# sara-nl/2D-VQ-AE-2

Hardware: AMD Instinct MI355X
Metric: patches/sec (VQAE.forward: encoder -> VQ -> decoder) (higher is better)
Workload: dtype f32; 1 GPU; BASELINE configs[1] (cfg B): batch 256/GPU of 256x256x3 fp32 -> 32x32 codes, K=256, D=128, full forward; global_batch=256, parallelism=patch-sharded x1

## Files before the change

2d-vq-ae-2_amd/csrc/handle.hip:

```cpp
#include "kernels.h"

#include <algorithm>
#include <cmath>
#include <cstdlib>
#include <map>
#include <mutex>
#include <set>
#include <string>
#include <unordered_map>
#include <utility>
#include <vector>

namespace vqae {
char* last_error_buf() {
    static thread_local char buf[512] = {0};
    return buf;
}

ProfState& prof_state() {
    static ProfState p;
    return p;
}

int set_max_dynamic_lds(const void* kernel, int bytes) {
// ... 100 lines not shown
    std::vector<void*> owned;
    float* buf[4] = {nullptr, nullptr, nullptr, nullptr};
    size_t buf_floats = 0;
    void* vq_ws = nullptr;
    size_t vq_ws_bytes = 0;
    float* loss_scratch = nullptr;
    int device = 0;
    bool has_encoder = false, has_decoder = false;
    bool fuse_trunk = true;
    bool t1_ready = false;
    bool up_conv_first = true;
    bool fuse_down = true;
    bool fuse_down16 = true;
    bool fuse_up16 = true;
    bool fuse_up_tail = true;
    bool use_wino = true;
    bool w43_split = true;
    void* idx_scratch = nullptr;
    size_t idx_scratch_bytes = 0;
    float* se_ws = nullptr;
    size_t se_ws_bytes = 0;
    size_t se_gate_off = 0;
};

namespace {

using TensorMap = std::unordered_map<std::string, const vqae_tensor*>;

int find(const TensorMap& tm, const std::string& name, int64_t numel, const float** out) {
    auto it = tm.find(name);
// ... 73 lines not shown
    const int dt = h->cfg.compute_dtype;
    const bool f32 = dt == VQAE_DT_F32, same = mode == MODE_SAME && cout == cin;
    int rc;
#define S_(field, nm) if ((rc = scalar(tm, pre + "." nm, &b->field))) return rc;
    S_(b1a, "bias1a") S_(b1b, "bias1b") S_(b2a, "bias2a") S_(b2b, "bias2b") S_(b3a, "bias3a") S_(b3b, "bias3b")
    S_(b4, "bias4") S_(scale, "scale")
    const bool wino = same && h->use_wino && vqae::wino_trunk_channels(cin, dt);
    const bool wino43 = wino && f32 && vqae::wino43_enabled() && vqae::wino43_channels(cin);
    const bool split = wino43 && h->w43_split && vqae::wino43_split_supported(cin);
    const bool tail = wino || (same && vqae::conv_trunk_tail_channels(cin));
    const bool trunk16 = same && !f32 && vqae::trunk16_channels(cin);
    const bool same8 = same && !f32 && vqae::same8_16_channels(cin);
    const bool down = mode == MODE_DOWN && cout == 2 * cin && h->fuse_down && vqae::down_block_channels(cin);
    const bool down16 = mode == MODE_DOWN && cout == 2 * cin && !f32 && h->fuse_down16 && vqae::down16_channels(cin);
    const bool up16 = mode == MODE_UP && cin == 2 * cout && !f32 && h->fuse_up16 && vqae::up16_channels(cin);

    const int k2 = mode == MODE_SAME ? 3 : (mode == MODE_DOWN ? 2 : 1);
    const float* p;
    if ((rc = find(tm, pre + ".branch_conv1.weight", (int64_t)b->br * cin, &p))) return rc;
    if ((rc = upload_packed(h, p, b->br, cin, 1, &b->w1))) return rc;
    if ((rc = find(tm, pre + ".branch_conv2.weight", (int64_t)b->br * b->br * k2 * k2, &p))) return rc;
    if ((rc = upload_packed(h, p, b->br, b->br, k2, &b->w2))) return rc;
    if (wino && (rc = upload_wino(h, p, cin, &b->wU))) return rc;
    if (wino43 && (rc = upload_wino43(h, p, cin, false, (void**)&b->wU43))) return rc;
    if (split && (rc = upload_wino43(h, p, cin, true, &b->wU43s))) return rc;
    if ((rc = find(tm, pre + ".branch_conv3.weight", (int64_t)cout * b->br, &p))) return rc;
    if ((rc = upload_packed(h, p, cout, b->br, 1, &b->w3))) return rc;
    if (mode != MODE_SAME) {
        S_(b1c, "bias1c") S_(b1d, "bias1d")
        const int ks = mode == MODE_DOWN ? 2 : 1;
// ... 15 lines not shown
    };
    auto pack_t16 = [&](const float* src, int taps, void** dst) {
        if (int r = dev_alloc(h, vqae::trunk16_weight_bytes(cin, taps), dst)) return r;
        return vqae::pack16_weight(src, cin, taps * cin, dt, *dst, nullptr);
    };
    auto pack_r16 = [&](const float* src, int rows, int K, void** dst) {
        if (int r = dev_alloc(h, vqae::down16_weight_bytes(rows, K), dst)) return r;
        return vqae::pack16_weight(src, rows, K, dt, *dst, nullptr);
    };
    if (tail && ((rc = frag_tail(b->w1, &b->w1f)) || (rc = frag_tail(b->w3, &b->w3f)))) return rc;
    if (split && ((rc = split3(b->w1, &b->w1s)) || (rc = split3(b->w3, &b->w3s)))) return rc;
    if (trunk16 && ((rc = pack_t16(b->w1, 1, &b->w1h)) || (rc = pack_t16(b->w2, 9, &b->w2h)) || (rc = pack_t16(b->w3, 1, &b->w3h)))) return rc;
    if (same8 && ((rc = pack_r16(b->w2, 8, 72, &b->w2h)) || (rc = pack_r16(b->w3, 8, 8, &b->w3h)))) return rc;
    if (down && ((rc = frag_rect(b->w1, cin, &b->w1f)) || (rc = frag_rect(b->w2, 4 * cout, &b->w2f)) ||
                 (rc = frag_rect(b->w3, cout, &b->w3f)) || (rc = frag_rect(b->wskip, 4 * cin, &b->wskf)))) return rc;
    if (down16 && ((rc = pack_r16(b->w1, cout, cin, &b->w1h)) || (rc = pack_r16(b->w2, cout, 4 * cout, &b->w2h)) ||
                   (rc = pack_r16(b->w3, cout, cout, &b->w3h)) || (rc = pack_r16(b->wskip, cout, 4 * cin, &b->wskh)))) return rc;
    if (up16 && ((rc = pack_t16(b->w1, 1, &b->w1h)) || (rc = pack_r16(b->w2, cin, cin, &b->w2h)) ||
                 (rc = pack_r16(b->w3, cout, cin, &b->w3h)) || (rc = pack_r16(b->wskip, cout, cin, &b->wskh)))) return rc;
    VQAE_HIP_CHECK(hipDeviceSynchronize());
    return VQAE_OK;
}

int bn_fold(const TensorMap& tm, const std::string& pre, int c, float eps, std::vector<float>* g, std::vector<float>* shift) {
    const float *gamma, *beta, *mean, *var;
    int rc;
    if ((rc = find(tm, pre + ".weight", c, &gamma)) || (rc = find(tm, pre + ".bias", c, &beta)) ||
        (rc = find(tm, pre + ".running_mean", c, &mean)) || (rc = find(tm, pre + ".running_var", c, &var))) return rc;
    g->resize(c); shift->resize(c);
    for (int i = 0; i < c; ++i) {
// ... 252 lines not shown
        out = R;
        break;
    case R_DOWN_FUSED:
        if ((rc = vqae::down_block(X, b.w1f, b.w2f, b.w3f, b.wskf, B, H, W, b.cin, b, dt, R, st))) return rc;
        out = R;
        break;
    case R_DOWN:
        if ((rc = conv(ConvCall(h, B, H, W, b.cin, b.cout, 2, 2, 0, VQAE_PAD_NONE).pre(VQAE_PRE_BIAS, b.b1c, 0.f).bias(b.b1d), X, b.wskip, nullptr, R, st))) return rc;
        if ((rc = run_conv1(h, b, B, H, W, X, P, st))) return rc;
        if ((rc = conv(ConvCall(h, B, H, W, b.br, b.br, 2, 2, 0, VQAE_PAD_NONE).act(b.b3a, b.b3b), P, b.w2, nullptr, Q, st))) return rc;
        if ((rc = conv(ConvCall(h, B, H / 2, W / 2, b.br, b.cout, 1, 1, 0, VQAE_PAD_NONE).scale_bias(b.scale, b.b4), Q, b.w3, R, R, st))) return rc;
        out = R;
        break;
    case R_UP_CONV_FIRST_TAIL:
    case R_UP_CONV_FIRST: {
        const ConvCall sk = ConvCall(h, B, H, W, b.cin, b.cout, 1, 1, 0, VQAE_PAD_NONE).pre(VQAE_PRE_BIAS, b.b1c, 0.f).bias(b.b1d);
        const ConvCall c2(h, B, H, W, b.br, b.br, 1, 1, 0, VQAE_PAD_NONE);
        if ((rc = conv(sk, X, b.wskip, nullptr, Q, st))) return rc;
        if (r == R_UP_CONV_FIRST_TAIL) {
            if ((rc = run_conv1(h, b, B, H, W, X, P, st))) return rc;
            if ((rc = conv(c2, P, b.w2, nullptr, R, st))) return rc;
            if ((rc = vqae::up_tail(R, Q, b.w3, B, H, W, b.br, b.cout, b.b3a, b.b3b, b.scale, b.b4, X, st))) return rc;
            break;
        }
        if ((rc = vqae_bicubic_up2_f32(Q, B, H, W, b.cout, 0.f, R, st))) return rc;
        if ((rc = run_conv1(h, b, B, H, W, X, P, st))) return rc;
        if ((rc = conv(c2, P, b.w2, nullptr, Q, st))) return rc;
        if ((rc = vqae_bicubic_up2_f32(Q, B, H, W, b.br, 0.f, P, st))) return rc;
        if ((rc = conv(ConvCall(h, B, 2 * H, 2 * W, b.br, b.cout, 1, 1, 0, VQAE_PAD_NONE).pre(VQAE_PRE_BIAS_ELU_BIAS, b.b3a, b.b3b).scale_bias(b.scale, b.b4),
                       P, b.w3, R, R, st))) return rc;
        out = R;
        break;
    }
    case R_UP16:
        if ((rc = vqae::trunk16_head(X, b.w1h, b.b1a, b.b1b, b.b2a, b.b2b, Q, (int64_t)B * H * W, b.cin, dt, true, st))) return rc;
        if ((rc = vqae::up16_block(X, Q, b.w2h, b.w3h, b.wskh, B, H, W, b.cin, b, dt, R, st))) return rc;
        out = R;
        break;
    default:
        if ((rc = vqae_bicubic_up2_f32(X, B, H, W, b.cin, b.b1c, P, st))) return rc;
        if ((rc = conv(ConvCall(h, B, 2 * H, 2 * W, b.cin, b.cout, 1, 1, 0, VQAE_PAD_NONE).bias(b.b1d), P, b.wskip, nullptr, R, st))) return rc;
        if ((rc = run_conv1(h, b, B, H, W, X, Q, st))) return rc;
        if ((rc = vqae_bicubic_up2_f32(Q, B, H, W, b.br, 0.f, P, st))) return rc;
        if ((rc = conv(ConvCall(h, B, 2 * H, 2 * W, b.br, b.br, 1, 1, 0, VQAE_PAD_NONE).act(b.b3a, b.b3b), P, b.w2, nullptr, Q, st))) return rc;
        if ((rc = conv(ConvCall(h, B, 2 * H, 2 * W, b.br, b.cout, 1, 1, 0, VQAE_PAD_NONE).scale_bias(b.scale, b.b4), Q, b.w3, R, R, st))) return rc;
        out = R;
// ... 159 lines not shown
        VQAE_REQUIRE(cfg->compute_dtype == VQAE_DT_F32, VQAE_ERR_UNSUPPORTED, "MBConv blocks run in fp32 only");
        VQAE_REQUIRE(cfg->expand_ratio >= 1 && cfg->se_divisor >= 1 && cfg->bn_eps > 0.f, VQAE_ERR_INVALID,
                     "MBConv: expand_ratio %d, se_divisor %d, bn_eps %g", cfg->expand_ratio, cfg->se_divisor, (double)cfg->bn_eps);
    }
    TensorMap tm;
    for (int i = 0; i < n_tensors; ++i) tm[tensors[i].name] = &tensors[i];

    vqae_handle* h = new vqae_handle();
    h->cfg = *cfg;
    if (hipGetDevice(&h->device) != hipSuccess) { delete h; return vqae::fail(VQAE_ERR_HIP, "hipGetDevice failed"); }
    h->fuse_trunk = vqae::env_int("VQAE_NO_TRUNK_FUSION", 0) == 0;
    h->up_conv_first = vqae::env_int("VQAE_NO_UP_REORDER", 0) == 0;
    h->use_wino = vqae::env_int("VQAE_NO_WINOGRAD", 0) == 0;
    h->w43_split = vqae::env_int("VQAE_W43_SPLIT", 1) != 0;
    h->fuse_up_tail = vqae::env_int("VQAE_NO_UP_TAIL_FUSION", 0) == 0;
    h->fuse_down = vqae::env_int("VQAE_NO_DOWN_FUSION", 0) == 0;
    h->fuse_down16 = vqae::env_int("VQAE_NO_DOWN16", 0) == 0;
    h->fuse_up16 = vqae::env_int("VQAE_NO_UP16", 0) == 0;
    h->fuse_stem16 = vqae::env_int("VQAE_NO_STEM16", 0) == 0;
    h->fuse_vq = vqae::env_int("VQAE_NO_VQ_FUSION", 0) == 0;
    h->C = cfg->stem << cfg->n_down;
    h->D = cfg->projection_dim > 0 ? cfg->projection_dim : h->C;
    h->K = cfg->num_embeddings;
    int rc = VQAE_OK;
    const float* p;
    auto bail = [&](int code) { vqae_destroy(h); return code; };

    const bool has_enc = tm.count("encoder.in_stem.weight") > 0;
    const bool has_dec = tm.count("decoder.out_stem.weight") > 0;
    if (!has_enc && !has_dec) return bail(vqae::fail(VQAE_ERR_NOT_FOUND, "neither encoder.* nor decoder.* tensors given"));
// ... 317 lines not shown
```

2d-vq-ae-2_amd/csrc/kernels.h:

```cpp
#pragma once
#include "common.h"

namespace vqae {

struct FixupScalars {
    float b1a, b1b, b2a, b2b, b3a, b3b, b4, scale, b1c, b1d;
};
static_assert(sizeof(FixupScalars) == 10 * sizeof(float), "FixupScalars is read as float[8] / float[10]");

struct NextConv1 {
    const void* w1 = nullptr;
    const void* w1s = nullptr;
    float b1a = 0.f, b1b = 0.f, b2a = 0.f, b2b = 0.f;
    void* t1_next = nullptr;
};

bool conv_trunk_tail_channels(int c);
int conv_tail_kslice(int dtype, int cin);
int conv_trunk_tail(const vqae_conv_args* a, const float* t1, const float* w2, const float* w3, float t_scale, float t_b4,
                    float* xio, const NextConv1& next, hipStream_t stream);

bool wino_trunk_channels(int c, int dtype);
bool wino_trunk_supported(int c, int h, int w, int dtype);
size_t wino_weight_floats(int c);
// ... 50 lines not shown

bool up16_channels(int c);
bool up16_supported(int c, int h, int w, int dtype);
int up16_block(const float* x, const float* t1, const void* w2h, const void* w3h, const void* wskh, int B, int H, int W, int c,
               const FixupScalars& s, int dtype, float* y, hipStream_t stream);

bool stem16_channels(int c0);
bool stem16_supported(int c0, int h, int w, int dtype);
size_t stem16_weight_bytes(int cin);
int stem16_pack_weight(const float* w_dev, int n_out, int cin, int dtype, void* out_dev, hipStream_t stream);
int istem16(const void* x, int x_kind, const float* mean255, const float* inv_std255, const void* wf, const float* bias, int B,
            int H, int W, int c0, float* y, int dtype, hipStream_t stream);
int ostem16(const float* x, const void* wf, const float* bias, int B, int H, int W, int c, float* y, int y_nchw, int dtype,
            hipStream_t stream);

bool up_tail_supported(int cb, int co);
int up_tail(const float* q, const float* s, const float* w3_packed, int B, int H, int W, int cb, int co, float b3a, float b3b,
            float scale, float b4, float* y, hipStream_t stream);
bool conv_small_k_supported(const vqae_conv_args* a);
int conv_small_k(const vqae_conv_args* a, const float* x, const float* w, const float* bias_vec, const float* residual,
                 float* y, hipStream_t stream);
int conv3x3_direct(const void* x, int x_kind, const float* mean255, const float* inv_std255, const float* w,
                   const float* bias, int B, int H, int W, int cin, int cout, float* y, int y_nchw, int dt,
                   hipStream_t stream);

int unstitch_tiles(const void* grid, int grid_dtype, const int32_t* rc, int n_tiles, int th, int tw, void* tiles,
                   int idx_dtype, int gh, int gw, hipStream_t stream);
int pixels_u8(const float* x, int layout, int B, int H, int W, const int32_t* rc, const float* mean255, const float* std255,
              uint8_t* out, int canvas_h, int canvas_w, hipStream_t stream);
int pixels_u8_level_check(const char* who, int H, int W, int level, bool canvas, int canvas_h, int canvas_w);
int pixels_u8_level(const float* x, int layout, int B, int H, int W, int level, const int32_t* rc, const float* mean255,
                    const float* std255, uint8_t* out, int canvas_h, int canvas_w, hipStream_t stream);

// ... 22 lines not shown
```

2d-vq-ae-2_amd/csrc/misc_kernels.hip:

```cpp
#include "kernels.h"
#include "mfma.h"

namespace {


template <int CIN, int COUT>
__global__ __launch_bounds__(256)
void conv3x3_direct_kernel(const void* __restrict__ xin, int x_kind, Norm3 nrm, const float* __restrict__ w,
                           const float* __restrict__ bias, int B, int H, int W, float* __restrict__ y, int y_nchw,
                           int dt) {
    __shared__ float ws[9 * CIN * COUT + COUT];
    for (int i = threadIdx.x; i < 9 * CIN * COUT; i += 256) {
        const int co = i % COUT, ci = (i / COUT) % CIN, tap = i / (COUT * CIN);
        ws[i] = vqae::round_dt(w[((int64_t)co * CIN + ci) * 9 + tap], dt);
    }
    for (int i = threadIdx.x; i < COUT; i += 256) ws[9 * CIN * COUT + i] = vqae::round_dt(bias[i], dt);
    __syncthreads();

    const int64_t npix = (int64_t)B * H * W;
    const int64_t pix = (int64_t)blockIdx.x * 256 + threadIdx.x;
    if (pix >= npix) return;
    const int hw = H * W;
    const int b = (int)(pix / hw), rem = (int)(pix - (int64_t)b * hw);
    const int oy = rem / W, ox = rem - oy * W;
// ... 109 lines not shown
            if (oy < 0 || oy >= OH) continue;
            const float* wy = a == 0 ? w25 : w75;
#pragma unroll
            for (int c = 0; c < 2; ++c) {
                const int ox = 2 * bj + 1 + c;
                if (ox < 0 || ox >= OW) continue;
                const float4* in = c == 0 ? ho : he;
                float4 out;
                out.x = in[0].x * wy[0]; out.y = in[0].y * wy[0]; out.z = in[0].z * wy[0]; out.w = in[0].w * wy[0];
#pragma unroll
                for (int r = 1; r < 4; ++r) {
                    out.x = out.x + in[r].x * wy[r]; out.y = out.y + in[r].y * wy[r];
                    out.z = out.z + in[r].z * wy[r]; out.w = out.w + in[r].w * wy[r];
                }
                y[(((int64_t)b * OH + oy) * OW + ox) * C4 + c4] = out;
            }
        }
    }
}

template <int CB, int CO>
__global__ __launch_bounds__(256)
void up_tail_kernel(const float4* __restrict__ q, const float4* __restrict__ sk, const float* __restrict__ w3, int B, int H,
                    int W, int tiles_x, int tiles_y, float b3a, float b3b, float scale, float b4, float* __restrict__ y) {
    constexpr int LB = CB + 4, LS = CO + 4, GB = CB / 4, GS = CO / 4, NG = GB + GS;
    constexpr int NTL = (CO + 15) / 16;
    static_assert(CB % 16 == 0 && CO % 4 == 0, "conv3 runs on 16x16x4 MFMA tiles");
    const float w75[4] = {-0.03515625f, 0.26171875f, 0.87890625f, -0.10546875f};
    const float w25[4] = {-0.10546875f, 0.87890625f, 0.26171875f, -0.03515625f};
    __shared__ __attribute__((aligned(16))) float Tb[128 * LB];
    __shared__ __attribute__((aligned(16))) float Ts[128 * LS];
    const int tid = threadIdx.x;
    float4 w3r[NTL][CB / 16];
#pragma unroll
    for (int nt = 0; nt < NTL; ++nt)
#pragma unroll
        for (int s_ = 0; s_ < CB / 16; ++s_) {
            const int co = 16 * nt + (tid & 15);
            w3r[nt][s_] = co < CO ? *reinterpret_cast<const float4*>(w3 + co * CB + 16 * s_ + 4 * ((tid & 63) >> 4)) : make_float4(0.f, 0.f, 0.f, 0.f);
        }
    const int OW = 2 * W, OH = 2 * H;
    const int n_tiles = B * tiles_x * tiles_y;
    for (int tile = blockIdx.x; tile < n_tiles; tile += gridDim.x) {
        const int txi = tile % tiles_x;
        const int tyi = (tile / tiles_x) % tiles_y;
        const int64_t b = tile / (tiles_x * tiles_y);
        const int bi0 = 2 * tyi - 1, bj0 = 16 * txi - 1;
        __syncthreads();
        for (int it = tid; it < 32 * NG; it += 256) {
            const int g = it % NG, blk = it / NG;
            const int bi = bi0 + (blk >> 4), bj = bj0 + (blk & 15);
            const bool branch = g < GB;
            const float4* src = branch ? q : sk;
            const int C4 = branch ? GB : GS, gg = branch ? g : g - GB;
            int xs[4], ys[4];
#pragma unroll
            for (int j = 0; j < 4; ++j) {
                int v = bj - 1 + j; xs[j] = v < 0 ? 0 : (v > W - 1 ? W - 1 : v);
                int u = bi - 1 + j; ys[j] = u < 0 ? 0 : (u > H - 1 ? H - 1 : u);
            }
            float4 ho[4], he[4];
#pragma unroll
            for (int r = 0; r < 4; ++r) {
                const float4* row = src + ((b * H + ys[r]) * W) * C4 + gg;
                float4 v[4];
#pragma unroll
                for (int j = 0; j < 4; ++j) v[j] = row[(int64_t)xs[j] * C4];
                ho[r].x = v[0].x * w25[0]; ho[r].y = v[0].y * w25[0]; ho[r].z = v[0].z * w25[0]; ho[r].w = v[0].w * w25[0];
                he[r].x = v[0].x * w75[0]; he[r].y = v[0].y * w75[0]; he[r].z = v[0].z * w75[0]; he[r].w = v[0].w * w75[0];
#pragma unroll
                for (int j = 1; j < 4; ++j) {
                    ho[r].x = __builtin_fmaf(v[j].x, w25[j], ho[r].x); ho[r].y = __builtin_fmaf(v[j].y, w25[j], ho[r].y);
                    ho[r].z = __builtin_fmaf(v[j].z, w25[j], ho[r].z); ho[r].w = __builtin_fmaf(v[j].w, w25[j], ho[r].w);
                    he[r].x = __builtin_fmaf(v[j].x, w75[j], he[r].x); he[r].y = __builtin_fmaf(v[j].y, w75[j], he[r].y);
                    he[r].z = __builtin_fmaf(v[j].z, w75[j], he[r].z); he[r].w = __builtin_fmaf(v[j].w, w75[j], he[r].w);
                }
            }
#pragma unroll
            for (int a = 0; a < 2; ++a) {
                const float* wy = a == 0 ? w25 : w75;
#pragma unroll
                for (int c = 0; c < 2; ++c) {
                    const float4* in = c == 0 ? ho : he;
                    float4 o;
                    o.x = in[0].x * wy[0]; o.y = in[0].y * wy[0]; o.z = in[0].z * wy[0]; o.w = in[0].w * wy[0];
#pragma unroll
                    for (int r = 1; r < 4; ++r) {
                        o.x = __builtin_fmaf(in[r].x, wy[r], o.x); o.y = __builtin_fmaf(in[r].y, wy[r], o.y);
                        o.z = __builtin_fmaf(in[r].z, wy[r], o.z); o.w = __builtin_fmaf(in[r].w, wy[r], o.w);
                    }
                    const int px = (2 * (blk >> 4) + a) * 32 + 2 * (blk & 15) + c;
                    if (branch) {
                        o.x = vqae::elu_act(o.x + b3a) + b3b; o.y = vqae::elu_act(o.y + b3a) + b3b;
                        o.z = vqae::elu_act(o.z + b3a) + b3b; o.w = vqae::elu_act(o.w + b3a) + b3b;
                        *reinterpret_cast<float4*>(Tb + px * LB + 4 * gg) = o;
                    } else {
                        *reinterpret_cast<float4*>(Ts + px * LS + 4 * gg) = o;
                    }
                }
            }
        }
        __syncthreads();
        {
            const int lane = tid & 63, wv = tid >> 6;
            const int li = lane & 15, q = lane >> 4;
#pragma unroll
            for (int gg = 0; gg < 2; ++gg) {
                const int px = 32 * wv + 16 * gg + li;
                const int oy = 2 * bi0 + 1 + (px >> 5), ox = 2 * bj0 + 1 + (px & 31);
                float4 tb[CB / 16];
#pragma unroll
                for (int s_ = 0; s_ < CB / 16; ++s_) tb[s_] = *reinterpret_cast<const float4*>(Tb + px * LB + 16 * s_ + 4 * q);
#pragma unroll
                for (int nt = 0; nt < NTL; ++nt) {
                    typedef float f32x4_t __attribute__((ext_vector_type(4)));
                    f32x4_t acc = {0.f, 0.f, 0.f, 0.f};
#pragma unroll
                    for (int s_ = 0; s_ < CB / 16; ++s_) {
                        const float4 wv4 = w3r[nt][s_];
                        acc = __builtin_amdgcn_mfma_f32_16x16x4f32(wv4.x, tb[s_].x, acc, 0, 0, 0);
                        acc = __builtin_amdgcn_mfma_f32_16x16x4f32(wv4.y, tb[s_].y, acc, 0, 0, 0);
                        acc = __builtin_amdgcn_mfma_f32_16x16x4f32(wv4.z, tb[s_].z, acc, 0, 0, 0);
                        acc = __builtin_amdgcn_mfma_f32_16x16x4f32(wv4.w, tb[s_].w, acc, 0, 0, 0);
                    }
                    if (oy >= 0 && oy < OH && ox >= 0 && ox < OW && 16 * nt + 4 * q < CO) {
                        const float4 sp = *reinterpret_cast<const float4*>(Ts + px * LS + 16 * nt + 4 * q);
                        float o[4];
                        const float sv[4] = {sp.x, sp.y, sp.z, sp.w};
#pragma unroll
                        for (int e = 0; e < 4; ++e) {
                            float tv = acc[e] * scale;
                            tv = tv + b4;
                            o[e] = tv + sv[e];
                        }
                        *reinterpret_cast<float4*>(y + ((b * OH + oy) * OW + ox) * CO + 16 * nt + 4 * q) = make_float4(o[0], o[1], o[2], o[3]);
                    }
                }
            }
        }
    }
}

__global__ __launch_bounds__(256)
void transpose_kernel(const float* __restrict__ in, int R, int S, float* __restrict__ out) {
    __shared__ float tile[32][33];
    const int64_t base = (int64_t)blockIdx.z * R * S;
    const int s0 = blockIdx.x * 32, r0 = blockIdx.y * 32;
    const int tx = threadIdx.x & 31, ty = threadIdx.x >> 5;
#pragma unroll
    for (int j = 0; j < 32; j += 8) {
        const int r = r0 + ty + j, s = s0 + tx;
        if (r < R && s < S) tile[ty + j][tx] = in[base + (int64_t)r * S + s];
// ... 187 lines not shown
        out[0] += r.x; out[1] += r.y; out[2] += r.z; out[3] += r.w;
    }
    if (p.has_act == VQAE_ACT_SILU) {
#pragma unroll
        for (int e = 0; e < 4; ++e) out[e] = out[e] / (1.0f + expf(-out[e]));
    } else if (p.has_act) {
#pragma unroll
        for (int e = 0; e < 4; ++e) out[e] = vqae::elu_act(out[e] + p.act_a) + p.act_b;
    }
    *reinterpret_cast<float4*>(p.y + o) = make_float4(out[0], out[1], out[2], out[3]);
}

}

namespace vqae {
bool up_tail_supported(int cb, int co) { return (cb == 64 && co == 32) || (cb == 32 && co == 16) || (cb == 16 && co == 8); }

int up_tail(const float* q, const float* s, const float* w3_packed, int B, int H, int W, int cb, int co, float b3a, float b3b,
            float scale, float b4, float* y, hipStream_t stream) {
    VQAE_REQUIRE(q && s && w3_packed && y, VQAE_ERR_INVALID, "up_tail: null pointer");
    VQAE_REQUIRE(up_tail_supported(cb, co), VQAE_ERR_UNSUPPORTED, "up_tail: channels %d -> %d", cb, co);
    if ((int64_t)B * H * W == 0) return VQAE_OK;
    const int tiles_x = (int)ceil_div(W + 1, 16), tiles_y = (int)ceil_div(H + 1, 2);
    const int64_t n_tiles = (int64_t)B * tiles_x * tiles_y;
    VQAE_REQUIRE(n_tiles < (1ll << 31), VQAE_ERR_UNSUPPORTED, "up_tail: too many tiles");
    const unsigned grid = (unsigned)std::min<int64_t>(n_tiles, 256 * 40);
    if (cb == 64) up_tail_kernel<64, 32><<<grid, 256, 0, stream>>>((const float4*)q, (const float4*)s, w3_packed, B, H, W, tiles_x, tiles_y, b3a, b3b, scale, b4, y);
    else if (cb == 32) up_tail_kernel<32, 16><<<grid, 256, 0, stream>>>((const float4*)q, (const float4*)s, w3_packed, B, H, W, tiles_x, tiles_y, b3a, b3b, scale, b4, y);
    else up_tail_kernel<16, 8><<<grid, 256, 0, stream>>>((const float4*)q, (const float4*)s, w3_packed, B, H, W, tiles_x, tiles_y, b3a, b3b, scale, b4, y);
    VQAE_LAUNCH_CHECK();
    return VQAE_OK;
}

bool conv_small_k_supported(const vqae_conv_args* a) {
    return a->cin == 8 && a->pad == 0 && a->ksize == a->stride && (a->ksize == 1 || a->ksize == 2) && a->cout % 4 == 0 &&
           a->cout <= 64 && a->pre_mode <= VQAE_PRE_BIAS_ELU_BIAS && a->in_h % a->ksize == 0 && a->in_w % a->ksize == 0;
}

int conv_small_k(const vqae_conv_args* a, const float* x, const float* w, const float* bias_vec, const float* residual,
                 float* y, hipStream_t stream) {
    SmallK p;
    p.x = x; p.w = w; p.bias_vec = bias_vec; p.residual = residual; p.y = y;
    p.H = a->in_h; p.W = a->in_w; p.Ho = a->in_h / a->ksize; p.Wo = a->in_w / a->ksize; p.cout = a->cout;
    p.M = (int64_t)a->batch * p.Ho * p.Wo;
    p.pre_mode = a->pre_mode; p.has_scale = a->has_scale; p.has_bias_s = a->has_bias_s; p.has_act = a->has_act; p.dt = a->dtype;
    p.pre_a = a->pre_a; p.pre_b = a->pre_b; p.scale = a->scale; p.bias_s = a->bias_s; p.act_a = a->act_a; p.act_b = a->act_b;
    const int64_t threads = p.M * (a->cout / 4);
    if (threads == 0) return VQAE_OK;
// ... 137 lines not shown
```

Measured before the change: 4513 patches/s.

## Fuse up-block head convs into one MFMA kernel and retile up_tail

Adds an up_head kernel that computes the skip 1x1 conv, branch conv1 and conv2 for the up block in one pass. The conv1 output stays in LDS, which removes the intermediate global round-trips and the separate launches. The up_tail kernel moves to a new file and is rewritten to tile by output pixels (8x16), loading an input window into LDS before the bicubic interpolation instead of re-reading neighbours per block. The non-tail path also reorders its buffers so the bicubic upsampling runs on the fused outputs. In exchange it adds more register-heavy kernels and more buffer aliasing, which could go wrong.

```diff
diff --git a/2d-vq-ae-2_amd/csrc/handle.hip b/2d-vq-ae-2_amd/csrc/handle.hip
--- a/2d-vq-ae-2_amd/csrc/handle.hip
+++ b/2d-vq-ae-2_amd/csrc/handle.hip
@@ -138,6 +138,7 @@
     bool fuse_down16 = true;
     bool fuse_up16 = true;
     bool fuse_up_tail = true;
+    bool fuse_up_head = true;
     bool use_wino = true;
     bool w43_split = true;
     void* idx_scratch = nullptr;
@@ -241,6 +242,7 @@
     const bool down = mode == MODE_DOWN && cout == 2 * cin && h->fuse_down && vqae::down_block_channels(cin);
     const bool down16 = mode == MODE_DOWN && cout == 2 * cin && !f32 && h->fuse_down16 && vqae::down16_channels(cin);
     const bool up16 = mode == MODE_UP && cin == 2 * cout && !f32 && h->fuse_up16 && vqae::up16_channels(cin);
+    const bool up_head = mode == MODE_UP && cin == 2 * cout && b->br == cin && f32 && h->up_conv_first && h->fuse_up_head && vqae::up_head_channels(cin);
 
     const int k2 = mode == MODE_SAME ? 3 : (mode == MODE_DOWN ? 2 : 1);
     const float* p;
@@ -286,6 +288,8 @@
     if (same8 && ((rc = pack_r16(b->w2, 8, 72, &b->w2h)) || (rc = pack_r16(b->w3, 8, 8, &b->w3h)))) return rc;
     if (down && ((rc = frag_rect(b->w1, cin, &b->w1f)) || (rc = frag_rect(b->w2, 4 * cout, &b->w2f)) ||
                  (rc = frag_rect(b->w3, cout, &b->w3f)) || (rc = frag_rect(b->wskip, 4 * cin, &b->wskf)))) return rc;
+    if (up_head && ((rc = frag(b->w1, cin, cin, 8, &b->w1f)) || (rc = frag(b->w2, cin, cin, 8, &b->w2f)) ||
+                    (rc = frag(b->wskip, std::max(cout, 32), cin, 8, &b->wskf)))) return rc;
     if (down16 && ((rc = pack_r16(b->w1, cout, cin, &b->w1h)) || (rc = pack_r16(b->w2, cout, 4 * cout, &b->w2h)) ||
                    (rc = pack_r16(b->w3, cout, cout, &b->w3h)) || (rc = pack_r16(b->wskip, cout, 4 * cin, &b->wskh)))) return rc;
     if (up16 && ((rc = pack_t16(b->w1, 1, &b->w1h)) || (rc = pack_r16(b->w2, cin, cin, &b->w2h)) ||
@@ -568,22 +572,22 @@
         break;
     case R_UP_CONV_FIRST_TAIL:
     case R_UP_CONV_FIRST: {
-        const ConvCall sk = ConvCall(h, B, H, W, b.cin, b.cout, 1, 1, 0, VQAE_PAD_NONE).pre(VQAE_PRE_BIAS, b.b1c, 0.f).bias(b.b1d);
-        const ConvCall c2(h, B, H, W, b.br, b.br, 1, 1, 0, VQAE_PAD_NONE);
-        if ((rc = conv(sk, X, b.wskip, nullptr, Q, st))) return rc;
+        if (b.w1f && b.w2f && b.wskf) {
+            if ((rc = vqae::up_head(X, b.w1f, b.w2f, b.wskf, (int64_t)B * H * W, b.cin, b, Q, R, st))) return rc;
+        } else {
+            const ConvCall sk = ConvCall(h, B, H, W, b.cin, b.cout, 1, 1, 0, VQAE_PAD_NONE).pre(VQAE_PRE_BIAS, b.b1c, 0.f).bias(b.b1d);
+            if ((rc = conv(sk, X, b.wskip, nullptr, Q, st))) return rc;
+            if ((rc = run_conv1(h, b, B, H, W, X, P, st))) return rc;
+            if ((rc = conv(ConvCall(h, B, H, W, b.br, b.br, 1, 1, 0, VQAE_PAD_NONE), P, b.w2, nullptr, R, st))) return rc;
+        }
         if (r == R_UP_CONV_FIRST_TAIL) {
-            if ((rc = run_conv1(h, b, B, H, W, X, P, st))) return rc;
-            if ((rc = conv(c2, P, b.w2, nullptr, R, st))) return rc;
             if ((rc = vqae::up_tail(R, Q, b.w3, B, H, W, b.br, b.cout, b.b3a, b.b3b, b.scale, b.b4, X, st))) return rc;
             break;
         }
-        if ((rc = vqae_bicubic_up2_f32(Q, B, H, W, b.cout, 0.f, R, st))) return rc;
-        if ((rc = run_conv1(h, b, B, H, W, X, P, st))) return rc;
-        if ((rc = conv(c2, P, b.w2, nullptr, Q, st))) return rc;
-        if ((rc = vqae_bicubic_up2_f32(Q, B, H, W, b.br, 0.f, P, st))) return rc;
+        if ((rc = vqae_bicubic_up2_f32(Q, B, H, W, b.cout, 0.f, X, st))) return rc;
+        if ((rc = vqae_bicubic_up2_f32(R, B, H, W, b.br, 0.f, P, st))) return rc;
         if ((rc = conv(ConvCall(h, B, 2 * H, 2 * W, b.br, b.cout, 1, 1, 0, VQAE_PAD_NONE).pre(VQAE_PRE_BIAS_ELU_BIAS, b.b3a, b.b3b).scale_bias(b.scale, b.b4),
-                       P, b.w3, R, R, st))) return rc;
-        out = R;
+                       P, b.w3, X, X, st))) return rc;
         break;
     }
     case R_UP16:
@@ -773,6 +777,7 @@
     h->use_wino = vqae::env_int("VQAE_NO_WINOGRAD", 0) == 0;
     h->w43_split = vqae::env_int("VQAE_W43_SPLIT", 1) != 0;
     h->fuse_up_tail = vqae::env_int("VQAE_NO_UP_TAIL_FUSION", 0) == 0;
+    h->fuse_up_head = vqae::env_int("VQAE_NO_UP_HEAD_FUSION", 0) == 0;
     h->fuse_down = vqae::env_int("VQAE_NO_DOWN_FUSION", 0) == 0;
     h->fuse_down16 = vqae::env_int("VQAE_NO_DOWN16", 0) == 0;
     h->fuse_up16 = vqae::env_int("VQAE_NO_UP16", 0) == 0;
diff --git a/2d-vq-ae-2_amd/csrc/kernels.h b/2d-vq-ae-2_amd/csrc/kernels.h
--- a/2d-vq-ae-2_amd/csrc/kernels.h
+++ b/2d-vq-ae-2_amd/csrc/kernels.h
@@ -88,9 +88,13 @@
 int ostem16(const float* x, const void* wf, const float* bias, int B, int H, int W, int c, float* y, int y_nchw, int dtype,
             hipStream_t stream);
 
+bool up_head_channels(int c);
+int up_head(const float* x, const float* w1f, const float* w2f, const float* wskf, int64_t M, int c, const FixupScalars& s,
+            float* q, float* r, hipStream_t stream);
 bool up_tail_supported(int cb, int co);
 int up_tail(const float* q, const float* s, const float* w3_packed, int B, int H, int W, int cb, int co, float b3a, float b3b,
             float scale, float b4, float* y, hipStream_t stream);
+
 bool conv_small_k_supported(const vqae_conv_args* a);
 int conv_small_k(const vqae_conv_args* a, const float* x, const float* w, const float* bias_vec, const float* residual,
                  float* y, hipStream_t stream);
diff --git a/2d-vq-ae-2_amd/csrc/misc_kernels.hip b/2d-vq-ae-2_amd/csrc/misc_kernels.hip
--- a/2d-vq-ae-2_amd/csrc/misc_kernels.hip
+++ b/2d-vq-ae-2_amd/csrc/misc_kernels.hip
@@ -147,128 +147,6 @@
                     out.z = out.z + in[r].z * wy[r]; out.w = out.w + in[r].w * wy[r];
                 }
                 y[(((int64_t)b * OH + oy) * OW + ox) * C4 + c4] = out;
-            }
-        }
-    }
-}
-
-template <int CB, int CO>
-__global__ __launch_bounds__(256)
-void up_tail_kernel(const float4* __restrict__ q, const float4* __restrict__ sk, const float* __restrict__ w3, int B, int H,
-                    int W, int tiles_x, int tiles_y, float b3a, float b3b, float scale, float b4, float* __restrict__ y) {
-    constexpr int LB = CB + 4, LS = CO + 4, GB = CB / 4, GS = CO / 4, NG = GB + GS;
-    constexpr int NTL = (CO + 15) / 16;
-    static_assert(CB % 16 == 0 && CO % 4 == 0, "conv3 runs on 16x16x4 MFMA tiles");
-    const float w75[4] = {-0.03515625f, 0.26171875f, 0.87890625f, -0.10546875f};
-    const float w25[4] = {-0.10546875f, 0.87890625f, 0.26171875f, -0.03515625f};
-    __shared__ __attribute__((aligned(16))) float Tb[128 * LB];
-    __shared__ __attribute__((aligned(16))) float Ts[128 * LS];
-    const int tid = threadIdx.x;
-    float4 w3r[NTL][CB / 16];
-#pragma unroll
-    for (int nt = 0; nt < NTL; ++nt)
-#pragma unroll
-        for (int s_ = 0; s_ < CB / 16; ++s_) {
-            const int co = 16 * nt + (tid & 15);
-            w3r[nt][s_] = co < CO ? *reinterpret_cast<const float4*>(w3 + co * CB + 16 * s_ + 4 * ((tid & 63) >> 4)) : make_float4(0.f, 0.f, 0.f, 0.f);
-        }
-    const int OW = 2 * W, OH = 2 * H;
-    const int n_tiles = B * tiles_x * tiles_y;
-    for (int tile = blockIdx.x; tile < n_tiles; tile += gridDim.x) {
-        const int txi = tile % tiles_x;
-        const int tyi = (tile / tiles_x) % tiles_y;
-        const int64_t b = tile / (tiles_x * tiles_y);
-        const int bi0 = 2 * tyi - 1, bj0 = 16 * txi - 1;
-        __syncthreads();
-        for (int it = tid; it < 32 * NG; it += 256) {
-            const int g = it % NG, blk = it / NG;
-            const int bi = bi0 + (blk >> 4), bj = bj0 + (blk & 15);
-            const bool branch = g < GB;
-            const float4* src = branch ? q : sk;
-            const int C4 = branch ? GB : GS, gg = branch ? g : g - GB;
-            int xs[4], ys[4];
-#pragma unroll
-            for (int j = 0; j < 4; ++j) {
-                int v = bj - 1 + j; xs[j] = v < 0 ? 0 : (v > W - 1 ? W - 1 : v);
-                int u = bi - 1 + j; ys[j] = u < 0 ? 0 : (u > H - 1 ? H - 1 : u);
-            }
-            float4 ho[4], he[4];
-#pragma unroll
-            for (int r = 0; r < 4; ++r) {
-                const float4* row = src + ((b * H + ys[r]) * W) * C4 + gg;
-                float4 v[4];
-#pragma unroll
-                for (int j = 0; j < 4; ++j) v[j] = row[(int64_t)xs[j] * C4];
-                ho[r].x = v[0].x * w25[0]; ho[r].y = v[0].y * w25[0]; ho[r].z = v[0].z * w25[0]; ho[r].w = v[0].w * w25[0];
-                he[r].x = v[0].x * w75[0]; he[r].y = v[0].y * w75[0]; he[r].z = v[0].z * w75[0]; he[r].w = v[0].w * w75[0];
-#pragma unroll
-                for (int j = 1; j < 4; ++j) {
-                    ho[r].x = __builtin_fmaf(v[j].x, w25[j], ho[r].x); ho[r].y = __builtin_fmaf(v[j].y, w25[j], ho[r].y);
-                    ho[r].z = __builtin_fmaf(v[j].z, w25[j], ho[r].z); ho[r].w = __builtin_fmaf(v[j].w, w25[j], ho[r].w);
-                    he[r].x = __builtin_fmaf(v[j].x, w75[j], he[r].x); he[r].y = __builtin_fmaf(v[j].y, w75[j], he[r].y);
-                    he[r].z = __builtin_fmaf(v[j].z, w75[j], he[r].z); he[r].w = __builtin_fmaf(v[j].w, w75[j], he[r].w);
-                }
-            }
-#pragma unroll
-            for (int a = 0; a < 2; ++a) {
-                const float* wy = a == 0 ? w25 : w75;
-#pragma unroll
-                for (int c = 0; c < 2; ++c) {
-                    const float4* in = c == 0 ? ho : he;
-                    float4 o;
-                    o.x = in[0].x * wy[0]; o.y = in[0].y * wy[0]; o.z = in[0].z * wy[0]; o.w = in[0].w * wy[0];
-#pragma unroll
-                    for (int r = 1; r < 4; ++r) {
-                        o.x = __builtin_fmaf(in[r].x, wy[r], o.x); o.y = __builtin_fmaf(in[r].y, wy[r], o.y);
-                        o.z = __builtin_fmaf(in[r].z, wy[r], o.z); o.w = __builtin_fmaf(in[r].w, wy[r], o.w);
-                    }
-                    const int px = (2 * (blk >> 4) + a) * 32 + 2 * (blk & 15) + c;
-                    if (branch) {
-                        o.x = vqae::elu_act(o.x + b3a) + b3b; o.y = vqae::elu_act(o.y + b3a) + b3b;
-                        o.z = vqae::elu_act(o.z + b3a) + b3b; o.w = vqae::elu_act(o.w + b3a) + b3b;
-                        *reinterpret_cast<float4*>(Tb + px * LB + 4 * gg) = o;
-                    } else {
-                        *reinterpret_cast<float4*>(Ts + px * LS + 4 * gg) = o;
-                    }
-                }
-            }
-        }
-        __syncthreads();
-        {
-            const int lane = tid & 63, wv = tid >> 6;
-            const int li = lane & 15, q = lane >> 4;
-#pragma unroll
-            for (int gg = 0; gg < 2; ++gg) {
-                const int px = 32 * wv + 16 * gg + li;
-                const int oy = 2 * bi0 + 1 + (px >> 5), ox = 2 * bj0 + 1 + (px & 31);
-                float4 tb[CB / 16];
-#pragma unroll
-                for (int s_ = 0; s_ < CB / 16; ++s_) tb[s_] = *reinterpret_cast<const float4*>(Tb + px * LB + 16 * s_ + 4 * q);
-#pragma unroll
-                for (int nt = 0; nt < NTL; ++nt) {
-                    typedef float f32x4_t __attribute__((ext_vector_type(4)));
-                    f32x4_t acc = {0.f, 0.f, 0.f, 0.f};
-#pragma unroll
-                    for (int s_ = 0; s_ < CB / 16; ++s_) {
-                        const float4 wv4 = w3r[nt][s_];
-                        acc = __builtin_amdgcn_mfma_f32_16x16x4f32(wv4.x, tb[s_].x, acc, 0, 0, 0);
-                        acc = __builtin_amdgcn_mfma_f32_16x16x4f32(wv4.y, tb[s_].y, acc, 0, 0, 0);
-                        acc = __builtin_amdgcn_mfma_f32_16x16x4f32(wv4.z, tb[s_].z, acc, 0, 0, 0);
-                        acc = __builtin_amdgcn_mfma_f32_16x16x4f32(wv4.w, tb[s_].w, acc, 0, 0, 0);
-                    }
-                    if (oy >= 0 && oy < OH && ox >= 0 && ox < OW && 16 * nt + 4 * q < CO) {
-                        const float4 sp = *reinterpret_cast<const float4*>(Ts + px * LS + 16 * nt + 4 * q);
-                        float o[4];
-                        const float sv[4] = {sp.x, sp.y, sp.z, sp.w};
-#pragma unroll
-                        for (int e = 0; e < 4; ++e) {
-                            float tv = acc[e] * scale;
-                            tv = tv + b4;
-                            o[e] = tv + sv[e];
-                        }
-                        *reinterpret_cast<float4*>(y + ((b * OH + oy) * OW + ox) * CO + 16 * nt + 4 * q) = make_float4(o[0], o[1], o[2], o[3]);
-                    }
-                }
             }
         }
     }
@@ -486,24 +364,6 @@
 }
 
 namespace vqae {
-bool up_tail_supported(int cb, int co) { return (cb == 64 && co == 32) || (cb == 32 && co == 16) || (cb == 16 && co == 8); }
-
-int up_tail(const float* q, const float* s, const float* w3_packed, int B, int H, int W, int cb, int co, float b3a, float b3b,
-            float scale, float b4, float* y, hipStream_t stream) {
-    VQAE_REQUIRE(q && s && w3_packed && y, VQAE_ERR_INVALID, "up_tail: null pointer");
-    VQAE_REQUIRE(up_tail_supported(cb, co), VQAE_ERR_UNSUPPORTED, "up_tail: channels %d -> %d", cb, co);
-    if ((int64_t)B * H * W == 0) return VQAE_OK;
-    const int tiles_x = (int)ceil_div(W + 1, 16), tiles_y = (int)ceil_div(H + 1, 2);
-    const int64_t n_tiles = (int64_t)B * tiles_x * tiles_y;
-    VQAE_REQUIRE(n_tiles < (1ll << 31), VQAE_ERR_UNSUPPORTED, "up_tail: too many tiles");
-    const unsigned grid = (unsigned)std::min<int64_t>(n_tiles, 256 * 40);
-    if (cb == 64) up_tail_kernel<64, 32><<<grid, 256, 0, stream>>>((const float4*)q, (const float4*)s, w3_packed, B, H, W, tiles_x, tiles_y, b3a, b3b, scale, b4, y);
-    else if (cb == 32) up_tail_kernel<32, 16><<<grid, 256, 0, stream>>>((const float4*)q, (const float4*)s, w3_packed, B, H, W, tiles_x, tiles_y, b3a, b3b, scale, b4, y);
-    else up_tail_kernel<16, 8><<<grid, 256, 0, stream>>>((const float4*)q, (const float4*)s, w3_packed, B, H, W, tiles_x, tiles_y, b3a, b3b, scale, b4, y);
-    VQAE_LAUNCH_CHECK();
-    return VQAE_OK;
-}
-
 bool conv_small_k_supported(const vqae_conv_args* a) {
     return a->cin == 8 && a->pad == 0 && a->ksize == a->stride && (a->ksize == 1 || a->ksize == 2) && a->cout % 4 == 0 &&
            a->cout <= 64 && a->pre_mode <= VQAE_PRE_BIAS_ELU_BIAS && a->in_h % a->ksize == 0 && a->in_w % a->ksize == 0;
diff --git a/2d-vq-ae-2_amd/csrc/up_fused.hip b/2d-vq-ae-2_amd/csrc/up_fused.hip
--- /dev/null
+++ b/2d-vq-ae-2_amd/csrc/up_fused.hip
@@ -0,0 +1,296 @@
+#include <type_traits>
+
+#include "kernels.h"
+#include "mfma.h"
+
+namespace {
+
+using namespace vqae;
+
+template <int C, int WRN, int WCN, int NIT>
+__device__ __forceinline__ void window_load(const float* __restrict__ img, int iy0, int jx0, int H, int W, int tid, f32x4 (&v)[NIT]) {
+    constexpr int G = C / 4, NITEM = WRN * WCN * G;
+#pragma unroll
+    for (int i = 0; i < NIT; ++i) {
+        int idx = tid + 256 * i;
+        idx = idx < NITEM ? idx : NITEM - 1;
+        const int wp = idx / G, g = idx % G;
+        int iy = iy0 - 2 + wp / WCN, ix = jx0 - 2 + wp % WCN;
+        iy = iy < 0 ? 0 : (iy > H - 1 ? H - 1 : iy);
+        ix = ix < 0 ? 0 : (ix > W - 1 ? W - 1 : ix);
+        v[i] = *reinterpret_cast<const f32x4*>(img + ((int64_t)iy * W + ix) * C + 4 * g);
+    }
+}
+
+template <int C, int WRN, int WCN, int L, int NIT>
+__device__ __forceinline__ void window_store(float* win, int tid, const f32x4 (&v)[NIT]) {
+    constexpr int G = C / 4, NITEM = WRN * WCN * G;
+#pragma unroll
+    for (int i = 0; i < NIT; ++i) {
+        const int idx = tid + 256 * i;
+        if (NITEM % 256 == 0 || idx < NITEM) *reinterpret_cast<f32x4*>(win + (idx / G) * L + 4 * (idx % G)) = v[i];
+    }
+}
+
+template <int CB, int CO>
+__global__ __launch_bounds__(256, CB == 64 ? 2 : 4)
+void up_tail_kernel(const float* __restrict__ q, const float* __restrict__ sk, const float* __restrict__ w3, int B, int H,
+                    int W, int tiles_x, int tiles_y, float b3a, float b3b, float scale, float b4, float* __restrict__ y) {
+    constexpr int TR = 8, TC = 16;
+    constexpr int WRN = TR / 2 + 4, WCN = TC / 2 + 4;
+    constexpr int LB = CB + 4, LS = CO + 4, GB = CB / 4, GS = CO / 4;
+    constexpr int NITEM = TC * (GB + GS), NI = (NITEM + 255) / 256;
+    constexpr int NLB = (WRN * WCN * GB + 255) / 256, NLS = (WRN * WCN * GS + 255) / 256;
+    constexpr int NTL = (CO + 15) / 16;
+    static_assert(CB % 16 == 0 && CO % 4 == 0, "conv3 runs on 16x16x4 MFMA tiles");
+    static_assert(TR * TC == 128 && WRN * WCN <= 128 && (TC * GB) % 64 == 0, "window under Tb / Ts; branch and skip items in separate waves");
+    const float w75[4] = {-0.03515625f, 0.26171875f, 0.87890625f, -0.10546875f};
+    const float w25[4] = {-0.10546875f, 0.87890625f, 0.26171875f, -0.03515625f};
+    __shared__ __attribute__((aligned(16))) float Tb[128 * LB];
+    __shared__ __attribute__((aligned(16))) float Ts[128 * LS];
+    const int tid = threadIdx.x;
+    float4 w3r[NTL][CB / 16];
+#pragma unroll
+    for (int nt = 0; nt < NTL; ++nt)
+#pragma unroll
+        for (int s_ = 0; s_ < CB / 16; ++s_) {
+            const int co = 16 * nt + (tid & 15);
+            w3r[nt][s_] = co < CO ? *reinterpret_cast<const float4*>(w3 + co * CB + 16 * s_ + 4 * ((tid & 63) >> 4)) : make_float4(0.f, 0.f, 0.f, 0.f);
+        }
+    const int OW = 2 * W, OH = 2 * H;
+    const int n_tiles = B * tiles_x * tiles_y;
+    for (int tile = blockIdx.x; tile < n_tiles; tile += gridDim.x) {
+        const int txi = tile % tiles_x;
+        const int tyi = (tile / tiles_x) % tiles_y;
+        const int64_t b = tile / (tiles_x * tiles_y);
+        const int oy0 = TR * tyi, ox0 = TC * txi;
+        f32x4 vb[NLB], vs[NLS];
+        window_load<CB, WRN, WCN, NLB>(q + b * H * W * CB, oy0 >> 1, ox0 >> 1, H, W, tid, vb);
+        window_load<CO, WRN, WCN, NLS>(sk + b * H * W * CO, oy0 >> 1, ox0 >> 1, H, W, tid, vs);
+        lds_barrier();
+        window_store<CB, WRN, WCN, LB, NLB>(Tb, tid, vb);
+        window_store<CO, WRN, WCN, LS, NLS>(Ts, tid, vs);
+        lds_barrier();
+        f32x4 h[NI][WRN];
+#pragma unroll
+        for (int ii = 0; ii < NI; ++ii) {
+            const int it = tid + 256 * ii;
+            if (NITEM % 256 != 0 && it >= NITEM) continue;
+            const bool branch = it < TC * GB;
+            const int c = it & (TC - 1), g = branch ? it / TC : it / TC - GB;
+            const int L = branch ? LB : LS;
+            const float* src = (branch ? Tb : Ts) + ((c >> 1) + (c & 1)) * L + 4 * g;
+            const float* wx = (c & 1) ? w25 : w75;
+            const float wx0 = wx[0], wx1 = wx[1], wx2 = wx[2], wx3 = wx[3];
+#pragma unroll
+            for (int wr = 0; wr < WRN; ++wr) {
+                const float* p = src + wr * WCN * L;
+                f32x4 a = *reinterpret_cast<const f32x4*>(p) * wx0;
+                a = __builtin_elementwise_fma(*reinterpret_cast<const f32x4*>(p + L), (f32x4){wx1, wx1, wx1, wx1}, a);
+                a = __builtin_elementwise_fma(*reinterpret_cast<const f32x4*>(p + 2 * L), (f32x4){wx2, wx2, wx2, wx2}, a);
+                a = __builtin_elementwise_fma(*reinterpret_cast<const f32x4*>(p + 3 * L), (f32x4){wx3, wx3, wx3, wx3}, a);
+                h[ii][wr] = a;
+            }
+        }
+        lds_barrier();
+#pragma unroll
+        for (int ii = 0; ii < NI; ++ii) {
+            const int it = tid + 256 * ii;
+            if (NITEM % 256 != 0 && it >= NITEM) continue;
+            const bool branch = it < TC * GB;
+            const int c = it & (TC - 1), g = branch ? it / TC : it / TC - GB;
+            float* dst = branch ? Tb + c * LB + 4 * g : Ts + c * LS + 4 * g;
+            const int L = branch ? LB : LS;
+#pragma unroll
+            for (int r = 0; r < TR; ++r) {
+                const int wrb = (r >> 1) + (r & 1);
+                const float* wy = (r & 1) ? w25 : w75;
+                f32x4 o = h[ii][wrb] * wy[0];
+#pragma unroll
+                for (int k = 1; k < 4; ++k) o = __builtin_elementwise_fma(h[ii][wrb + k], (f32x4){wy[k], wy[k], wy[k], wy[k]}, o);
+                if (branch) {
+#pragma unroll
+                    for (int e = 0; e < 4; ++e) o[e] = elu_act(o[e] + b3a) + b3b;
+                }
+                *reinterpret_cast<f32x4*>(dst + r * TC * L) = o;
+            }
+        }
+        lds_barrier();
+        {
+            const int lane = tid & 63, wv = tid >> 6;
+            const int li = lane & 15, qd = lane >> 4;
+#pragma unroll
+            for (int gg = 0; gg < 2; ++gg) {
+                const int px = 32 * wv + 16 * gg + li;
+                const int oy = oy0 + (px >> 4), ox = ox0 + (px & 15);
+                float4 tb[CB / 16];
+#pragma unroll
+                for (int s_ = 0; s_ < CB / 16; ++s_) tb[s_] = *reinterpret_cast<const float4*>(Tb + px * LB + 16 * s_ + 4 * qd);
+#pragma unroll
+                for (int nt = 0; nt < NTL; ++nt) {
+                    f32x4 acc = {0.f, 0.f, 0.f, 0.f};
+#pragma unroll
+                    for (int s_ = 0; s_ < CB / 16; ++s_) {
+                        const float4 wv4 = w3r[nt][s_];
+                        acc = __builtin_amdgcn_mfma_f32_16x16x4f32(wv4.x, tb[s_].x, acc, 0, 0, 0);
+                        acc = __builtin_amdgcn_mfma_f32_16x16x4f32(wv4.y, tb[s_].y, acc, 0, 0, 0);
+                        acc = __builtin_amdgcn_mfma_f32_16x16x4f32(wv4.z, tb[s_].z, acc, 0, 0, 0);
+                        acc = __builtin_amdgcn_mfma_f32_16x16x4f32(wv4.w, tb[s_].w, acc, 0, 0, 0);
+                    }
+                    if (oy < OH && ox < OW && 16 * nt + 4 * qd < CO) {
+                        const float4 sp = *reinterpret_cast<const float4*>(Ts + px * LS + 16 * nt + 4 * qd);
+                        float o[4];
+                        const float sv[4] = {sp.x, sp.y, sp.z, sp.w};
+#pragma unroll
+                        for (int e = 0; e < 4; ++e) {
+                            float tv = acc[e] * scale;
+                            tv = tv + b4;
+                            o[e] = tv + sv[e];
+                        }
+                        *reinterpret_cast<float4*>(y + ((b * OH + oy) * OW + ox) * CO + 16 * nt + 4 * qd) = make_float4(o[0], o[1], o[2], o[3]);
+                    }
+                }
+            }
+        }
+    }
+}
+
+struct UpHeadK {
+    const float* __restrict__ x;
+    const float* __restrict__ w1;
+    const float* __restrict__ w2;
+    const float* __restrict__ wsk;
+    float* __restrict__ q;
+    float* __restrict__ r;
+    int64_t M;
+    FixupScalars s;
+};
+
+template <int C>
+__global__ __launch_bounds__(256, 2)
+void up_head_kernel(const UpHeadK p) {
+    constexpr int CO = C / 2;
+    constexpr int KU = C / 8;
+    constexpr int NT = C / 32, NTS = (CO + 31) / 32;
+    constexpr int LD = C + 4;
+    constexpr int WR = 4;
+    extern __shared__ __attribute__((aligned(16))) float lds[];
+    const int tid = threadIdx.x;
+    const int lane = tid & 63;
+    const int wave = __builtin_amdgcn_readfirstlane(tid >> 6);
+    const int li = lane & 31, hh = lane >> 5;
+    const int64_t m = (int64_t)blockIdx.x * 128 + 32 * wave + li;
+    const bool m_ok = m < p.M;
+
+    f32x4 xin[KU];
+    {
+        const float* src = p.x + (m_ok ? m : p.M - 1) * C + 4 * hh;
+#pragma unroll
+        for (int u = 0; u < KU; ++u) xin[u] = *reinterpret_cast<const f32x4*>(src + 8 * u);
+    }
+    auto gemm = [&](const float* __restrict__ w, auto ntiles, auto&& operand, auto&& epilogue) {
+        constexpr int N = decltype(ntiles)::value * KU;
+        static_assert(N >= WR, "the ring's first loads stay inside the matrix");
+        const float* wl = w + 4 * lane;
+        f32x4 wq[WR];
+#pragma unroll
+        for (int j = 0; j < WR; ++j) wq[j] = *reinterpret_cast<const f32x4*>(wl + 256 * j);
+        f32x16 acc;
+#pragma unroll
+        for (int j = 0; j < N; ++j) {
+            const int ct = j / KU, u = j % KU;
+            if (u == 0) {
+#pragma unroll
+                for (int r = 0; r < 16; ++r) acc[r] = 0.f;
+            }
+            const f32x4 wv = wq[j % WR];
+            if (j + WR < N) wq[j % WR] = *reinterpret_cast<const f32x4*>(wl + 256 * (j + WR));
+            const f32x4 v = operand(u);
+#pragma unroll
+            for (int r = 0; r < 4; ++r) acc = __builtin_amdgcn_mfma_f32_32x32x2f32(wv[r], v[r], acc, 0, 0, 0);
+            if (u == KU - 1) epilogue(ct, acc);
+        }
+    };
+    gemm(p.wsk, std::integral_constant<int, NTS>(), [&](int u) { return xin[u] + p.s.b1c; }, [&](int ct, const f32x16& acc) {
+        float* dst = p.q + m * CO + 32 * ct + 4 * hh;
+#pragma unroll
+        for (int g = 0; g < 4; ++g) {
+            if (32 * ct + 8 * g >= CO) continue;
+            f32x4 o;
+#pragma unroll
+            for (int e = 0; e < 4; ++e) o[e] = acc[4 * g + e] + p.s.b1d;
+            if (m_ok) *reinterpret_cast<f32x4*>(dst + 8 * g) = o;
+        }
+    });
+#pragma unroll
+    for (int u = 0; u < KU; ++u)
+#pragma unroll
+        for (int e = 0; e < 4; ++e) xin[u][e] = elu_act(xin[u][e] + p.s.b1a) + p.s.b1b;
+    float* const trow = lds + (32 * wave + li) * LD + 4 * hh;
+    gemm(p.w1, std::integral_constant<int, NT>(), [&](int u) { return xin[u]; }, [&](int ct, const f32x16& acc) {
+#pragma unroll
+        for (int g = 0; g < 4; ++g) {
+            f32x4 o;
+#pragma unroll
+            for (int e = 0; e < 4; ++e) o[e] = elu_act(acc[4 * g + e] + p.s.b2a) + p.s.b2b;
+            *reinterpret_cast<f32x4*>(trow + 32 * ct + 8 * g) = o;
+        }
+    });
+    gemm(p.w2, std::integral_constant<int, NT>(), [&](int u) { return *reinterpret_cast<const f32x4*>(trow + 8 * u); },
+         [&](int ct, const f32x16& acc) {
+        float* dst = p.r + m * C + 32 * ct + 4 * hh;
+#pragma unroll
+        for (int g = 0; g < 4; ++g) {
+            const f32x4 o = {acc[4 * g], acc[4 * g + 1], acc[4 * g + 2], acc[4 * g + 3]};
+            if (m_ok) *reinterpret_cast<f32x4*>(dst + 8 * g) = o;
+        }
+    });
+}
+
+template <int C>
+int launch_up_head(const UpHeadK& k, hipStream_t stream) {
+    constexpr int lds_bytes = 128 * (C + 4) * 4;
+    if (int rc = vqae::set_max_dynamic_lds((const void*)up_head_kernel<C>, lds_bytes)) return rc;
+    up_head_kernel<C><<<(unsigned)ceil_div(k.M, 128), 256, lds_bytes, stream>>>(k);
+    VQAE_LAUNCH_CHECK();
+    return VQAE_OK;
+}
+
+}
+
+namespace vqae {
+
+bool up_head_channels(int c) { return c == 32 || c == 64 || c == 128; }
+
+int up_head(const float* x, const float* w1f, const float* w2f, const float* wskf, int64_t M, int c, const FixupScalars& s,
+            float* q, float* r, hipStream_t stream) {
+    if (M == 0) return VQAE_OK;
+    VQAE_REQUIRE(x && w1f && w2f && wskf && q && r, VQAE_ERR_INVALID, "up_head: null pointer");
+    VQAE_REQUIRE(up_head_channels(c), VQAE_ERR_UNSUPPORTED, "up_head: C = %d", c);
+    VQAE_REQUIRE(M > 0 && M < (1ll << 31) * 128, VQAE_ERR_UNSUPPORTED, "up_head: too many pixels");
+    UpHeadK k;
+    k.x = x; k.w1 = w1f; k.w2 = w2f; k.wsk = wskf; k.q = q; k.r = r; k.M = M; k.s = s;
+    if (c == 32) return launch_up_head<32>(k, stream);
+    if (c == 64) return launch_up_head<64>(k, stream);
+    return launch_up_head<128>(k, stream);
+}
+
+bool up_tail_supported(int cb, int co) { return (cb == 64 && co == 32) || (cb == 32 && co == 16) || (cb == 16 && co == 8); }
+
+int up_tail(const float* q, const float* s, const float* w3_packed, int B, int H, int W, int cb, int co, float b3a, float b3b,
+            float scale, float b4, float* y, hipStream_t stream) {
+    VQAE_REQUIRE(q && s && w3_packed && y, VQAE_ERR_INVALID, "up_tail: null pointer");
+    VQAE_REQUIRE(up_tail_supported(cb, co), VQAE_ERR_UNSUPPORTED, "up_tail: channels %d -> %d", cb, co);
+    if ((int64_t)B * H * W == 0) return VQAE_OK;
+    const int tiles_x = (int)ceil_div(2 * W, 16), tiles_y = (int)ceil_div(2 * H, 8);
+    const int64_t n_tiles = (int64_t)B * tiles_x * tiles_y;
+    VQAE_REQUIRE(n_tiles < (1ll << 31), VQAE_ERR_UNSUPPORTED, "up_tail: too many tiles");
+    const unsigned grid = (unsigned)std::min<int64_t>(n_tiles, 256 * 40);
+    if (cb == 64) up_tail_kernel<64, 32><<<grid, 256, 0, stream>>>(q, s, w3_packed, B, H, W, tiles_x, tiles_y, b3a, b3b, scale, b4, y);
+    else if (cb == 32) up_tail_kernel<32, 16><<<grid, 256, 0, stream>>>(q, s, w3_packed, B, H, W, tiles_x, tiles_y, b3a, b3b, scale, b4, y);
+    else up_tail_kernel<16, 8><<<grid, 256, 0, stream>>>(q, s, w3_packed, B, H, W, tiles_x, tiles_y, b3a, b3b, scale, b4, y);
+    VQAE_LAUNCH_CHECK();
+    return VQAE_OK;
+}
+
+}
```

Result: faster. 4599 patches/s, median of 6 (+1.9%).
